# turian/inverse-audio-synthesis

Measured on AMD Instinct MI355X. Metric: audio-seconds rendered+lossed/sec (whole node), batch=128 4s@44.1kHz, higher is better.
Workload: dtype f32; 1 GPU; BASELINE configs[1]: torchsynth-style Voice render + PQMF(3) analysis + mel-L1 loss, batch 128 x 4 s @ 44100 Hz per GPU; batch_per_gpu=128, samples_per_voice=176400, launch=hipgraph, streams=5, pipelined=True

## Files before the change

inverse-audio-synthesis_amd/csrc/voice_ctrl_kernels.hip:

```cpp
#define IAS_CTL_NO_LIBM
#include "voice_math.h"
#include "wave_ops.h"
#include "voice_table.h"

#define CS_THREADS 256
#define CS_WAVES (CS_THREADS / 64)
#define CS_KERNEL __global__ __launch_bounds__(CS_THREADS) __attribute__((amdgpu_num_vgpr(28)))

__constant__ IasParamRange c_cs_table[IAS_NPARAMS] = IAS_PARAM_TABLE_INIT;
__device__ const double g_cs_tab[IAS_CTL_TAB_DOUBLES] = IAS_CTL_TAB_INIT;

__device__ __forceinline__ void cs_stage_table(double* s_tab) {
  for (int i = threadIdx.x; i < IAS_CTL_TAB_DOUBLES; i += CS_THREADS) s_tab[i] = g_cs_tab[i];
}
__device__ __forceinline__ float cs_mapped(const float* __restrict__ params01, int b, int idx, const double* s_tab) {
  const IasParamRange r = c_cs_table[idx];
  return ias_map_param(params01[(size_t)b * IAS_NPARAMS + idx], (float)r.lo, (float)r.span, (float)r.curve, r.symmetric, s_tab);
}
__device__ __forceinline__ int cs_adsr_base(int a) {
  switch (a) {
    case 0: return IAS_P_ADSR_1_ATTACK;
    case 1: return IAS_P_ADSR_2_ATTACK;
    case 2: return IAS_P_LFO_1_AMP_ADSR_ATTACK;
    case 3: return IAS_P_LFO_2_AMP_ADSR_ATTACK;
    case 4: return IAS_P_LFO_1_RATE_ADSR_ATTACK;
    default: return IAS_P_LFO_2_RATE_ADSR_ATTACK;
  }
}

CS_KERNEL void voice_env_slim_kernel(const float* __restrict__ params01, float* __restrict__ sig, int Tc, float control_rate) {
  __shared__ __attribute__((aligned(16))) double s_tab[IAS_CTL_TAB_DOUBLES];
  __shared__ float s_p[8];
  const int a = blockIdx.x, b = blockIdx.y, tid = threadIdx.x;
  cs_stage_table(s_tab);
  __syncthreads();
  if (tid < 5) s_p[tid] = cs_mapped(params01, b, cs_adsr_base(a) + tid, s_tab);
  if (tid == 5) s_p[5] = cs_mapped(params01, b, IAS_P_KEYBOARD_DURATION, s_tab);
  __syncthreads();
  IasAdsr e;
  e.attack = s_p[0]; e.decay = s_p[1]; e.sustain = s_p[2]; e.release = s_p[3]; e.alpha = s_p[4];
  const float note_on = s_p[5], eps = (float)IAS_EPS;
  if (tid == 0) s_p[6] = ias_adsr_heads(e, note_on, control_rate, eps, s_tab).decay_head;
  if (tid == 64) s_p[7] = ias_adsr_heads(e, note_on, control_rate, eps, s_tab).release_head;
  __syncthreads();
  IasAdsrHeads heads;
  heads.decay_head = s_p[6]; heads.release_head = s_p[7];
  float* out = sig + ((size_t)b * 8 + a) * Tc;
  for (int t = tid; t < Tc; t += CS_THREADS) out[t] = ias_adsr_headed(t, e, note_on, control_rate, eps, heads, s_tab);
}

CS_KERNEL void voice_lfo_slim_kernel(const float* __restrict__ params01, float* __restrict__ sig,
                                     float* __restrict__ dbg ,
                                     int Tc, float control_rate) {
  extern __shared__ __attribute__((aligned(16))) double cs_smem[];
  double* s_tab = cs_smem;
  double* s_sum = s_tab + IAS_CTL_TAB_DOUBLES;
  __shared__ double s_wtot[CS_WAVES];
  __shared__ float s_q[8];
  __shared__ float s_mode[8];
  const int l = blockIdx.x, b = blockIdx.y, tid = threadIdx.x, lane = tid & 63, wave = tid >> 6;
  const int qbase = (l == 0) ? IAS_P_LFO_1_FREQUENCY : IAS_P_LFO_2_FREQUENCY;
  cs_stage_table(s_tab);
  __syncthreads();
  if (tid < 8) s_q[tid] = cs_mapped(params01, b, qbase + tid, s_tab);
  __syncthreads();
  if (tid < 5) s_mode[tid] = ias_pow_ctl(s_q[3 + tid], IAS_LFO_EXPONENT_F, s_tab);
  const float freq = s_q[0], depth = s_q[1], phi = s_q[2];
  const float* rate_env = sig + ((size_t)b * 8 + 4 + l) * Tc;
  const float* amp_env = sig + ((size_t)b * 8 + 2 + l) * Tc;

  const int per_wave = ((Tc + CS_WAVES - 1) / CS_WAVES + 63) / 64 * 64;
  const int t_begin = min(wave * per_wave, Tc), t_end = min(t_begin + per_wave, Tc);
  double carry = 0.0;
  for (int t0 = t_begin; t0 < t_end; t0 += 64) {
    const int t = t0 + lane;
    double inc = 0.0;
    if (t < t_end) inc = (double)ias_lfo_inc(freq, depth, rate_env[t], control_rate);
    const double sc = wave_incl_scan(inc, lane) + carry;
    carry = __shfl(sc, 63, 64);
    if (t < t_end) s_sum[t] = sc;
  }
  if (lane == 0) s_wtot[wave] = carry;
  __syncthreads();
  double base = 0.0;
  for (int w = 0; w < wave; ++w) base += s_wtot[w];
  float mode[5];
  {
    const float sm = (float)((double)s_mode[0] + (double)s_mode[1] + (double)s_mode[2] + (double)s_mode[3] + (double)s_mode[4]);
#pragma unroll
    for (int k = 0; k < 5; ++k) mode[k] = ias_div(s_mode[k], sm);
  }
  float* out = sig + ((size_t)b * 8 + 6 + l) * Tc;
  for (int t = t_begin + lane; t < t_end; t += 64) {
    const double ph = base + s_sum[t];
    const float arg = ias_add((float)ph, phi);
    const float o = ias_mul(ias_lfo_shape_mix(arg, mode, s_tab), amp_env[t]);
    out[t] = o;
    if (dbg != nullptr) {
      dbg[((size_t)b * 10 + 6 + l) * Tc + t] = arg;
      dbg[((size_t)b * 10 + 8 + l) * Tc + t] = o;
    }
  }
}

CS_KERNEL void voice_modmix_slim_kernel(const float* __restrict__ params01, const float* __restrict__ sig,
                                        float* __restrict__ ctrl, IasVoiceConst* __restrict__ vconst,
                                        float* __restrict__ dbg, int Tc) {
  __shared__ __attribute__((aligned(16))) double s_tab[IAS_CTL_TAB_DOUBLES];
  __shared__ float s_w[20];
  __shared__ float s_p[IAS_NPARAMS];
  const int b = blockIdx.y, tid = threadIdx.x;
  cs_stage_table(s_tab);
  __syncthreads();
  if (tid < 20) s_w[tid] = cs_mapped(params01, b, IAS_P_MOD_MATRIX_ADSR_1_TO_VCO_1_PITCH + tid, s_tab);
  if (blockIdx.x == 0 && tid >= 64 && tid < 64 + IAS_NPARAMS) s_p[tid - 64] = cs_mapped(params01, b, tid - 64, s_tab);
  __syncthreads();
  const float* sb = sig + (size_t)b * 8 * Tc;
  const int t = blockIdx.x * CS_THREADS + tid;
  if (t < Tc) {
    const float e0 = sb[t], e1 = sb[Tc + t], l0 = sb[6 * Tc + t], l1 = sb[7 * Tc + t];
    float* out = ctrl + (size_t)b * IAS_NCTRL * Tc;
#pragma unroll
    for (int j = 0; j < IAS_NCTRL; ++j)
      out[j * Tc + t] = ias_dot4_cr(s_w[j], s_w[5 + j], s_w[10 + j], s_w[15 + j], e0, e1, l0, l1);
    if (dbg != nullptr) {
#pragma unroll
      for (int r = 0; r < 6; ++r) dbg[((size_t)b * 10 + r) * Tc + t] = sb[r * Tc + t];
    }
  }
  if (blockIdx.x == 0 && tid == 0) {
    const float* p = s_p;
    const float midi_f0 = p[IAS_P_KEYBOARD_MIDI_F0];
    IasVoiceConst vc;
    vc.f0_1 = ias_add(midi_f0, p[IAS_P_VCO_1_TUNING]);
    vc.depth_1 = p[IAS_P_VCO_1_MOD_DEPTH];
    vc.phi_1 = p[IAS_P_VCO_1_INITIAL_PHASE];
    vc.f0_2 = ias_add(midi_f0, p[IAS_P_VCO_2_TUNING]);
    vc.depth_2 = p[IAS_P_VCO_2_MOD_DEPTH];
    vc.phi_2 = p[IAS_P_VCO_2_INITIAL_PHASE];
    vc.kpart = ias_partials_k(midi_f0, vc.depth_2, s_tab);
    vc.shape = p[IAS_P_VCO_2_SHAPE];
    vc.shape_gain = ias_sub(1.0f, ias_div(vc.shape, 2.0f));
    vc.lvl0 = p[IAS_P_MIXER_VCO_1];
    vc.lvl1 = p[IAS_P_MIXER_VCO_2];
    vc.lvl2 = p[IAS_P_MIXER_NOISE];
    vc.pad[0] = vc.pad[1] = vc.pad[2] = vc.pad[3] = 0.0f;
    vconst[b] = vc;
  }
}

bool ias_voice_control_slim_ok(int Tc, int control_rate) {
  return Tc <= 4096 && (double)Tc / (double)control_rate <= 600.0;
}
int ias_voice_control_slim_launch(const float* params01, float* ctrl, void* vconst, float* sig, float* dbg, int B, int Tc,
                                  int control_rate, hipStream_t stream) {
  const size_t lds = sizeof(double) * (IAS_CTL_TAB_DOUBLES + (size_t)Tc);
  hipLaunchKernelGGL(voice_env_slim_kernel, dim3(6, B), dim3(CS_THREADS), 0, stream, params01, sig, Tc, (float)control_rate);
  hipLaunchKernelGGL(voice_lfo_slim_kernel, dim3(2, B), dim3(CS_THREADS), lds, stream, params01, sig, dbg, Tc, (float)control_rate);
  hipLaunchKernelGGL(voice_modmix_slim_kernel, dim3((Tc + CS_THREADS - 1) / CS_THREADS, B), dim3(CS_THREADS), 0, stream, params01,
                     (const float*)sig, ctrl, (IasVoiceConst*)vconst, dbg, Tc);
  return hipGetLastError() == hipSuccess ? IAS_OK : IAS_ERR_LAUNCH;
}
```

Measured before the change: 3.493 million audio-s/s.

## Fuse ADSR envelope and LFO kernels into one chained control kernel

Merges the envelope kernel and the LFO kernel into a single launch of 4 blocks per voice. Each LFO block computes its own rate and amp envelopes, keeps them in LDS and feeds them straight into the phase scan. The other two blocks write only the two VCO envelopes. This drops one kernel launch and the global round trip of the envelope rows, at the cost of more LDS per block, possibly a larger dynamic-LDS attribute, and serial envelope work inside the LFO blocks. Uniform parameters are also forced into scalar registers via readfirstlane.

After: 3.594 million audio-s/s, median of 6. +2.9%, better.

```diff
diff --git a/inverse-audio-synthesis_amd/csrc/voice_ctrl_kernels.hip b/inverse-audio-synthesis_amd/csrc/voice_ctrl_kernels.hip
--- a/inverse-audio-synthesis_amd/csrc/voice_ctrl_kernels.hip
+++ b/inverse-audio-synthesis_amd/csrc/voice_ctrl_kernels.hip
@@ -17,6 +17,9 @@
   const IasParamRange r = c_cs_table[idx];
   return ias_map_param(params01[(size_t)b * IAS_NPARAMS + idx], (float)r.lo, (float)r.span, (float)r.curve, r.symmetric, s_tab);
 }
+__device__ __forceinline__ float cs_uniform(float x) {
+  return __int_as_float(__builtin_amdgcn_readfirstlane(__float_as_int(x)));
+}
 __device__ __forceinline__ int cs_adsr_base(int a) {
   switch (a) {
     case 0: return IAS_P_ADSR_1_ATTACK;
@@ -28,46 +31,70 @@
   }
 }
 
-CS_KERNEL void voice_env_slim_kernel(const float* __restrict__ params01, float* __restrict__ sig, int Tc, float control_rate) {
-  __shared__ __attribute__((aligned(16))) double s_tab[IAS_CTL_TAB_DOUBLES];
-  __shared__ float s_p[8];
-  const int a = blockIdx.x, b = blockIdx.y, tid = threadIdx.x;
-  cs_stage_table(s_tab);
-  __syncthreads();
-  if (tid < 5) s_p[tid] = cs_mapped(params01, b, cs_adsr_base(a) + tid, s_tab);
-  if (tid == 5) s_p[5] = cs_mapped(params01, b, IAS_P_KEYBOARD_DURATION, s_tab);
-  __syncthreads();
-  IasAdsr e;
-  e.attack = s_p[0]; e.decay = s_p[1]; e.sustain = s_p[2]; e.release = s_p[3]; e.alpha = s_p[4];
-  const float note_on = s_p[5], eps = (float)IAS_EPS;
-  if (tid == 0) s_p[6] = ias_adsr_heads(e, note_on, control_rate, eps, s_tab).decay_head;
-  if (tid == 64) s_p[7] = ias_adsr_heads(e, note_on, control_rate, eps, s_tab).release_head;
-  __syncthreads();
-  IasAdsrHeads heads;
-  heads.decay_head = s_p[6]; heads.release_head = s_p[7];
-  float* out = sig + ((size_t)b * 8 + a) * Tc;
-  for (int t = tid; t < Tc; t += CS_THREADS) out[t] = ias_adsr_headed(t, e, note_on, control_rate, eps, heads, s_tab);
+static size_t cs_chain_lds(int Tc) {
+  return sizeof(double) * (IAS_CTL_TAB_DOUBLES + (size_t)Tc) + sizeof(float) * 2 * (size_t)Tc;
 }
 
-CS_KERNEL void voice_lfo_slim_kernel(const float* __restrict__ params01, float* __restrict__ sig,
-                                     float* __restrict__ dbg ,
-                                     int Tc, float control_rate) {
+CS_KERNEL void voice_chain_slim_kernel(const float* __restrict__ params01, float* __restrict__ sig,
+                                       float* __restrict__ dbg ,
+                                       int Tc, float control_rate) {
   extern __shared__ __attribute__((aligned(16))) double cs_smem[];
   double* s_tab = cs_smem;
   double* s_sum = s_tab + IAS_CTL_TAB_DOUBLES;
+  float* s_row = reinterpret_cast<float*>(s_sum + Tc);
   __shared__ double s_wtot[CS_WAVES];
-  __shared__ float s_q[8];
+  __shared__ float s_p[19];
+  __shared__ float s_head[4];
   __shared__ float s_mode[8];
-  const int l = blockIdx.x, b = blockIdx.y, tid = threadIdx.x, lane = tid & 63, wave = tid >> 6;
-  const int qbase = (l == 0) ? IAS_P_LFO_1_FREQUENCY : IAS_P_LFO_2_FREQUENCY;
+  const int b = blockIdx.y, tid = threadIdx.x;
+  const bool is_lfo = blockIdx.x < 2;
+  const int l = blockIdx.x;
+  const int n_env = is_lfo ? 2 : 1;
+  const int row0 = is_lfo ? 4 + l : (int)blockIdx.x - 2, row1 = 2 + l;
+  const float eps = (float)IAS_EPS;
   cs_stage_table(s_tab);
   __syncthreads();
-  if (tid < 8) s_q[tid] = cs_mapped(params01, b, qbase + tid, s_tab);
+  {
+    int idx = -1;
+    if (tid < 5 * n_env) idx = cs_adsr_base(tid < 5 ? row0 : row1) + (tid < 5 ? tid : tid - 5);
+    else if (tid == 10) idx = IAS_P_KEYBOARD_DURATION;
+    else if (is_lfo && tid >= 11 && tid < 19) idx = ((l == 0) ? IAS_P_LFO_1_FREQUENCY : IAS_P_LFO_2_FREQUENCY) + (tid - 11);
+    if (idx >= 0) s_p[tid] = cs_mapped(params01, b, idx, s_tab);
+  }
   __syncthreads();
-  if (tid < 5) s_mode[tid] = ias_pow_ctl(s_q[3 + tid], IAS_LFO_EXPONENT_F, s_tab);
-  const float freq = s_q[0], depth = s_q[1], phi = s_q[2];
-  const float* rate_env = sig + ((size_t)b * 8 + 4 + l) * Tc;
-  const float* amp_env = sig + ((size_t)b * 8 + 2 + l) * Tc;
+  const float note_on = s_p[10];
+  if (tid < 64) {
+    if (tid < 2 * n_env) {
+      const float* q = s_p + 5 * (tid >> 1);
+      IasAdsr e; e.attack = q[0]; e.decay = q[1]; e.sustain = q[2]; e.release = q[3]; e.alpha = q[4];
+      const IasAdsrHeads h = ias_adsr_heads(e, note_on, control_rate, eps, s_tab);
+      s_head[tid] = (tid & 1) ? h.release_head : h.decay_head;
+    }
+  } else if (tid < 128) {
+    if (is_lfo && tid < 64 + 5) s_mode[tid - 64] = ias_pow_ctl(s_p[11 + 3 + tid - 64], IAS_LFO_EXPONENT_F, s_tab);
+  }
+  __syncthreads();
+#pragma unroll 1
+  for (int k = 0; k < n_env; ++k) {
+    const float* q = s_p + 5 * k;
+    IasAdsr e;
+    e.attack = cs_uniform(q[0]); e.decay = cs_uniform(q[1]); e.sustain = cs_uniform(q[2]); e.release = cs_uniform(q[3]);
+    e.alpha = cs_uniform(q[4]);
+    IasAdsrHeads heads; heads.decay_head = cs_uniform(s_head[2 * k]); heads.release_head = cs_uniform(s_head[2 * k + 1]);
+    float* out = sig + ((size_t)b * 8 + (k == 0 ? row0 : row1)) * Tc;
+    float* keep = s_row + (size_t)k * Tc;
+    for (int t = tid; t < Tc; t += CS_THREADS) {
+      const float v = ias_adsr_headed(t, e, note_on, control_rate, eps, heads, s_tab);
+      out[t] = v;
+      if (is_lfo) keep[t] = v;
+    }
+  }
+  if (!is_lfo) return;
+  __syncthreads();
+  const float freq = s_p[11], depth = s_p[12];
+  const float* rate_env = s_row;
+  const float* amp_env = s_row + Tc;
+  const int wave = __builtin_amdgcn_readfirstlane(tid >> 6), lane = __lane_id();
 
   const int per_wave = ((Tc + CS_WAVES - 1) / CS_WAVES + 63) / 64 * 64;
   const int t_begin = min(wave * per_wave, Tc), t_end = min(t_begin + per_wave, Tc);
@@ -84,6 +111,7 @@
   __syncthreads();
   double base = 0.0;
   for (int w = 0; w < wave; ++w) base += s_wtot[w];
+  const float phi = s_p[13];
   float mode[5];
   {
     const float sm = (float)((double)s_mode[0] + (double)s_mode[1] + (double)s_mode[2] + (double)s_mode[3] + (double)s_mode[4]);
@@ -154,9 +182,11 @@
 }
 int ias_voice_control_slim_launch(const float* params01, float* ctrl, void* vconst, float* sig, float* dbg, int B, int Tc,
                                   int control_rate, hipStream_t stream) {
-  const size_t lds = sizeof(double) * (IAS_CTL_TAB_DOUBLES + (size_t)Tc);
-  hipLaunchKernelGGL(voice_env_slim_kernel, dim3(6, B), dim3(CS_THREADS), 0, stream, params01, sig, Tc, (float)control_rate);
-  hipLaunchKernelGGL(voice_lfo_slim_kernel, dim3(2, B), dim3(CS_THREADS), lds, stream, params01, sig, dbg, Tc, (float)control_rate);
+  const size_t lds = cs_chain_lds(Tc);
+  if (lds > 64 * 1024 &&
+      hipFuncSetAttribute((const void*)voice_chain_slim_kernel, hipFuncAttributeMaxDynamicSharedMemorySize, (int)cs_chain_lds(4096)) != hipSuccess)
+    return IAS_ERR_LAUNCH;
+  hipLaunchKernelGGL(voice_chain_slim_kernel, dim3(4, B), dim3(CS_THREADS), lds, stream, params01, sig, dbg, Tc, (float)control_rate);
   hipLaunchKernelGGL(voice_modmix_slim_kernel, dim3((Tc + CS_THREADS - 1) / CS_THREADS, B), dim3(CS_THREADS), 0, stream, params01,
                      (const float*)sig, ctrl, (IasVoiceConst*)vconst, dbg, Tc);
   return hipGetLastError() == hipSuccess ? IAS_OK : IAS_ERR_LAUNCH;
```
